# graphcore-research/bess-kge

Measured on AMD Instinct MI355X. Metric: positive+negative triples scored/sec, higher is better.
Workload: dtype f32; 1 GPU; ogbl-biokg-shaped ComplEx d=256 fp32 (W=512), 93,773 entities per shard, n_shard=1, S=4096 positives x 256 per-triple negatives per GPU per step, EmbeddingMoving, mode=score (gather+score+loss); negatives_per_triple=256, mode=score, collectives=none

## Files before the change

bess-kge_amd/csrc/common.h:

```cpp
#pragma once

#include <hip/hip_fp16.h>
#include <hip/hip_runtime.h>
#include <stdint.h>

#include <type_traits>
#include <utility>

#include "../../include/besskge_hip.h"

namespace bess {

int fail(int code, const char* fmt, ...);
int check_launch(const char* what);

#define BESS_REQUIRE(cond, ...)                          \
    do {                                                 \
        if (!(cond)) return ::bess::fail(BESS_EINVAL, __VA_ARGS__); \
    } while (0)

inline hipStream_t as_stream(void* s) { return reinterpret_cast<hipStream_t>(s); }

inline int64_t ceil_div(int64_t a, int64_t b) { return (a + b - 1) / b; }

// ... 75 lines not shown
                   const CountArgs* count = nullptr);

typedef _Float16 half_t;

template <typename T>
__device__ __forceinline__ float to_f32(T v) {
    return static_cast<float>(v);
}

template <typename T, int VEC>
struct VecLoad {
    typedef T vec_t __attribute__((ext_vector_type(VEC)));
    __device__ __forceinline__ static void load(const T* __restrict__ p, float (&out)[VEC]) {
        vec_t v = *reinterpret_cast<const vec_t*>(p);
#pragma unroll
        for (int i = 0; i < VEC; ++i) out[i] = static_cast<float>(v[i]);
    }
};
template <typename T>
struct VecLoad<T, 1> {
    __device__ __forceinline__ static void load(const T* __restrict__ p, float (&out)[1]) {
        out[0] = static_cast<float>(*p);
    }
};

template <typename T, int VEC>
__device__ __forceinline__ void load_chunk(const T* __restrict__ row, int c, int nch, float (&out)[VEC]) {
    VecLoad<T, VEC>::load(row + min(c, nch - 1) * VEC, out);
    const bool live = c < nch;
#pragma unroll
    for (int i = 0; i < VEC; ++i) out[i] = live ? out[i] : 0.f;
}

template <typename T, int VEC>
__device__ __forceinline__ void load_chunk_clamped(const T* __restrict__ row, int c, int nch, float (&out)[VEC]) {
    VecLoad<T, VEC>::load(row + min(c, nch - 1) * VEC, out);
}

__device__ __forceinline__ float row16_allreduce_sum(float v) {
#define BESS_DPP_ROR(x, n)                                                                     \
    __builtin_bit_cast(float, __builtin_amdgcn_update_dpp(0, __builtin_bit_cast(int, (x)),     \
                                                           0x120 | (n), 0xf, 0xf, false))
    v += BESS_DPP_ROR(v, 8);
    v += BESS_DPP_ROR(v, 4);
    v += BESS_DPP_ROR(v, 2);
    v += BESS_DPP_ROR(v, 1);
#undef BESS_DPP_ROR
    return v;
}

__device__ __forceinline__ float wave_allreduce_sum(float v) {
    v = row16_allreduce_sum(v);
    v += __shfl_xor(v, 16, 64);
    v += __shfl_xor(v, 32, 64);
    return v;
}
__device__ __forceinline__ float wave_allreduce_max(float v) {
#pragma unroll
    for (int m = 32; m >= 1; m >>= 1) v = fmaxf(v, __shfl_xor(v, m, 64));
    return v;
}

__device__ __forceinline__ float sgnf(float x) {
    return (x > 0.f) ? 1.f : ((x < 0.f) ? -1.f : 0.f);
}

__device__ __forceinline__ void store_agent(float* p, float v) {
    __hip_atomic_store(p, v, __ATOMIC_RELAXED, __HIP_MEMORY_SCOPE_AGENT);
}
__device__ __forceinline__ float load_agent(const float* p) {
    return __hip_atomic_load(p, __ATOMIC_RELAXED, __HIP_MEMORY_SCOPE_AGENT);
}
__device__ __forceinline__ void release_to_agent() { asm volatile("s_waitcnt vmcnt(0)" ::: "memory"); }
__device__ __forceinline__ bool last_workgroup_ticket(int32_t* counters) {
    const int grid = static_cast<int>(gridDim.x), sub = static_cast<int>(blockIdx.x) & 15;
    const int members = (grid - sub + 15) >> 4;
    int32_t* mine = counters + 32 * (1 + sub);
    if (__hip_atomic_fetch_add(mine, 1, __ATOMIC_RELAXED, __HIP_MEMORY_SCOPE_AGENT) != members - 1) return false;
    __hip_atomic_store(mine, 0, __ATOMIC_RELAXED, __HIP_MEMORY_SCOPE_AGENT);
    if (__hip_atomic_fetch_add(counters, 1, __ATOMIC_RELAXED, __HIP_MEMORY_SCOPE_AGENT) != min(grid, 16) - 1) return false;
    __hip_atomic_store(counters, 0, __ATOMIC_RELAXED, __HIP_MEMORY_SCOPE_AGENT);
    return true;
}


constexpr float SGN_PRESCALE = 1.2676506002282294e30f;
__device__ __forceinline__ float sgn_prescaled(float d_scaled) {
    return __builtin_amdgcn_fmed3f(d_scaled, -1.f, 1.f);
}

struct WordJobs {
    uint32_t* dst[BESS_MAX_WORD_JOBS];
    const uint32_t* src[BESS_MAX_WORD_JOBS];
    uint32_t value[BESS_MAX_WORD_JOBS];
    int64_t first[BESS_MAX_WORD_JOBS + 1];
    int n;
};
__device__ __forceinline__ void run_word_jobs(const WordJobs& J, int block, int n_blocks, int threads) {
    const int64_t total = J.first[J.n];
    const int64_t stride = static_cast<int64_t>(n_blocks) * threads;
    for (int64_t i = static_cast<int64_t>(block) * threads + threadIdx.x; i < total; i += stride) {
        int j = 0;
#pragma unroll
        for (int k = 1; k < BESS_MAX_WORD_JOBS; ++k) j += (k < J.n && i >= J.first[k]) ? 1 : 0;
        const int64_t off = i - J.first[j];
        J.dst[j][off] = J.src[j] ? J.src[j][off] + J.value[j] : J.value[j];
    }
}
int make_word_jobs(int32_t n_jobs, void* const* job_dst, const void* const* job_src, const uint32_t* job_value,
                   const int64_t* job_words, WordJobs* J, int64_t* words, const char* who);

static __global__ __launch_bounds__(256) void k_fill_words(uint32_t* __restrict__ p, uint32_t v, int64_t n) {
    for (int64_t i = blockIdx.x * 256ll + threadIdx.x; i < n; i += 256ll * gridDim.x) p[i] = v;
}
inline hipError_t fill_words_async(void* p, uint32_t v, int64_t n_words, hipStream_t st) {
    if (n_words <= 0) return hipSuccess;
#ifdef BESS_PROBE_MEMSET_NODES
    if (v == 0u || v == 0xffffffffu) return hipMemsetAsync(p, static_cast<int>(v & 0xffu), sizeof(uint32_t) * n_words, st);
#endif
    int64_t blocks = (n_words + 255) / 256;
    blocks = blocks > 2048 ? 2048 : blocks;
    k_fill_words<<<static_cast<unsigned>(blocks), 256, 0, st>>>(static_cast<uint32_t*>(p), v, n_words);
    return hipGetLastError();
}

__device__ __forceinline__ float lp_term(float d, float p) { return p == 2.f ? d * d : powf(fabsf(d), p); }
__device__ __forceinline__ float lp_root(float acc, float p) { return p == 2.f ? sqrtf(acc) : powf(acc, 1.f / p); }
__device__ __forceinline__ float lp_dterm(float d, float p) {
    return p == 2.f ? d : copysignf(powf(fabsf(d), p - 1.f), d);
}
__device__ __forceinline__ float lp_inv(float norm, float p) {
    return norm > 0.f ? (p == 2.f ? 1.f / norm : powf(norm, 1.f - p)) : 0.f;
}

template <typename T>
__device__ __forceinline__ const T* row_ptr(const T* base, const int32_t* idx, int64_t i, int width) {
    const int64_t r = idx ? static_cast<int64_t>(idx[i]) : i;
    return base + r * width;
}

template <typename T_, int VEC_, int IT_>
struct RowClass {
    using T = T_;
    static constexpr int VEC = VEC_, IT = IT_;
};
template <int... V>
using Ints = std::integer_sequence<int, V...>;
struct NativeRows {
    using f32_vecs = Ints<4, 1>;
    using f16_vecs = Ints<8, 2, 1>;
    using its = Ints<1, 2, 4, 8, 16>;
};
struct PartRows {
    using f32_vecs = Ints<4, 1>;
    using f16_vecs = Ints<4, 1>;
    using its = Ints<1, 2, 4, 8>;
};
template <typename T, int VEC, typename F, int... ITS>
bool row_class_by_it(int it, F& f, Ints<ITS...>) {
    return ((it <= ITS ? (f(RowClass<T, VEC, ITS>{}), true) : false) || ...);
}
template <typename T, typename ITS, typename F, int... VECS>
bool row_class_by_vec(int vec, int it, F& f, Ints<VECS...>) {
    return ((vec == VECS && row_class_by_it<T, VECS>(it, f, ITS{})) || ...);
}
template <typename Policy, typename F>
// ... 60 lines not shown
```

bess-kge_amd/csrc/loss.hip:

```cpp
#include "common.h"
#include "loss_rows.h"

namespace bess {

__global__ __launch_bounds__(256) void k_mask_scores(float* __restrict__ neg, int64_t n_triple,
                                                     int64_t n_neg, int64_t ld, int diag_step, int ht,
                                                     int ppp, const uint8_t* __restrict__ mask,
                                                     int64_t mask_rows, int64_t mask_cols) {
    const int64_t total = n_triple * n_neg;
    const int cut = ppp / 2;
    for (int64_t t = blockIdx.x * 256ll + threadIdx.x; t < total; t += 256ll * gridDim.x) {
        const int64_t s = t / n_neg;
        const int64_t j = t - s * n_neg;
        const int64_t blk = ppp > 0 ? s / ppp : 0;
        const int p = ppp > 0 ? static_cast<int>(s - blk * ppp) : 0;
        bool kill = false;
        if (diag_step > 0) {
            const int64_t qpos = ht ? (blk * cut + (p % cut)) : s;
            kill = (j == static_cast<int64_t>(diag_step) * qpos);
        }
        const int64_t mj = j - (n_neg - mask_cols);
        if (mask && mj >= 0) {
            int64_t mrow = s;
            if (mask_rows == 1) mrow = 0;
            else if (mask_rows == 2) mrow = (p >= cut) ? 1 : 0;
            kill = mask[mrow * mask_cols + mj] == 0;
        }
        if (kill) neg[s * ld + j] += BESS_BAD_NEGATIVE_SCORE;
    }
}

template <int KIND, bool ADV, bool GRAD, int CH>
__global__ __launch_bounds__(256) void k_loss_rows(bess_loss_desc l, const float* __restrict__ pos,
                                                   const float* __restrict__ neg, int64_t n_triple,
                                                   int64_t n_neg, int64_t ld_neg,
                                                   const float* __restrict__ weight,
                                                   int64_t weight_len, float* __restrict__ row_loss,
                                                   float* __restrict__ d_pos,
                                                   float* __restrict__ d_neg, int64_t ld_dneg,
                                                   float* __restrict__ row_norm, int32_t* __restrict__ counter,
                                                   float* __restrict__ loss) {
    const int64_t s = blockIdx.x * 4ll + (threadIdx.x >> 6);
    if (s < n_triple)
        loss_row<KIND, ADV, GRAD, CH>(l, pos, neg, s, n_neg, ld_neg, weight, weight_len, row_loss, d_pos, d_neg, ld_dneg,
                                      row_norm);
    if (!counter) return;
    __shared__ float part[256];
    __shared__ int last;
    release_to_agent();
    __syncthreads();
    if (threadIdx.x == 0) last = last_workgroup_ticket(counter);
    __syncthreads();
    if (!last) return;
    float acc = 0.f;
    for (int64_t i = threadIdx.x; i < n_triple; i += 256) acc += load_agent(row_loss + i);
    part[threadIdx.x] = acc;
    __syncthreads();
    for (int h = 128; h > 0; h >>= 1) {
        if (threadIdx.x < h) part[threadIdx.x] += part[threadIdx.x + h];
        __syncthreads();
    }
    if (threadIdx.x == 0) loss[0] = part[0];
}

__global__ __launch_bounds__(256) void k_ranks_from_scores(const float* __restrict__ pos,
                                                           const float* __restrict__ cand, int64_t n_row,
                                                           int64_t n_cand, int64_t ld, int mode, int worst_inf,
                                                           float* __restrict__ rank) {
    const int lane = threadIdx.x & 63;
    const int64_t s = blockIdx.x * 4ll + (threadIdx.x >> 6);
    if (s >= n_row) return;
    float p = pos[s];
    if (p != p) p = -INFINITY;
    const float* row = cand + s * ld;
    float gt = 0.f, ge = 0.f;
    for (int64_t j = lane; j < n_cand; j += 64) {
        const float c = row[j];
        gt += (c > p) ? 1.f : 0.f;
        ge += (c >= p) ? 1.f : 0.f;
    }
    gt = wave_allreduce_sum(gt);
    ge = wave_allreduce_sum(ge);
    if (lane == 0) {
        const float n = static_cast<float>(n_cand);
        float better;
        bool worst;
        if (mode == 0) { better = gt; worst = gt == n; }
        else if (mode == 1) { better = ge; worst = ge == n; }
        else { better = 0.5f * (gt + ge); worst = (gt == n) || (ge == n); }
        rank[s] = (worst_inf && worst) ? INFINITY : 1.f + better;
    }
}

__global__ __launch_bounds__(256) void k_ranks_from_indices(const int64_t* __restrict__ truth,
                                                            const int64_t* __restrict__ cand, int64_t n_row,
                                                            int64_t n_cand, int worst_inf,
                                                            float* __restrict__ rank) {
    const int64_t s = blockIdx.x * 256ll + threadIdx.x;
    if (s >= n_row) return;
    const int64_t t = truth[s];
    float r = worst_inf ? INFINITY : static_cast<float>(n_cand + 1);
    for (int64_t j = n_cand - 1; j >= 0; --j)
        if (cand[s * n_cand + j] == t) r = static_cast<float>(j + 1);
    rank[s] = r;
}

__global__ __launch_bounds__(1024) void k_sum_rows(const float* __restrict__ row_loss, int64_t n,
                                                   float* __restrict__ loss) {
    __shared__ float part[1024];
    float acc = 0.f;
    for (int64_t i = threadIdx.x; i < n; i += 1024) acc += row_loss[i];
    part[threadIdx.x] = acc;
    __syncthreads();
    for (int s = 512; s > 0; s >>= 1) {
        if (threadIdx.x < s) part[threadIdx.x] += part[threadIdx.x + s];
        __syncthreads();
    }
    if (threadIdx.x == 0) loss[0] = part[0];
}

static int loss_chunks(bool grad, const float* neg, int64_t N, int64_t ld, const float* dn, int64_t ldd) {
    const bool vec = N % 4 == 0 && ld % 4 == 0 && reinterpret_cast<uintptr_t>(neg) % 16 == 0 &&
                     (!grad || (ldd % 4 == 0 && reinterpret_cast<uintptr_t>(dn) % 16 == 0));
    if (!vec) return 0;
    if (N > 256 * 24) return -1;
    return N <= 256 * 4 ? 4 : N <= 256 * 12 ? 12 : 24;
}

}

using namespace bess;

extern "C" int bess_mask_scores(float* neg, int64_t n_triple, int64_t n_neg, int64_t ld,
                                int32_t diag_step, int32_t ht, int32_t ppp, const uint8_t* mask,
                                int64_t mask_rows, int64_t mask_cols, void* stream) {
    BESS_REQUIRE(n_triple >= 0 && n_neg >= 0 && ld >= n_neg, "mask_scores: bad sizes");
    if (n_triple == 0 || n_neg == 0) return BESS_OK;
    BESS_REQUIRE(neg, "mask_scores: NULL scores");
    BESS_REQUIRE(diag_step >= 0, "mask_scores: negative diag_step");
// ... 101 lines not shown
```

bess-kge_amd/csrc/prepare.hip:

```cpp
#include "common.h"
#include "loss_rows.h"

namespace bess {

struct TripleArgs {
    const void* head_base;
    const int32_t* head_idx;
    const void* tail_base;
    const int32_t* tail_idx;
    const void* rel_table;
    const int32_t* rel_idx;
    int64_t n;
    int W;
    int Wr;
    int norm_p;
};

template <typename T, int SCORER>
__device__ __forceinline__ void triple_fwd_body(const TripleArgs& a, int64_t s, int lane, float* __restrict__ out) {
    const T* h = row_ptr(static_cast<const T*>(a.head_base), a.head_idx, s, a.W);
    const T* t = row_ptr(static_cast<const T*>(a.tail_base), a.tail_idx, s, a.W);
    const T* r = static_cast<const T*>(a.rel_table) + static_cast<int64_t>(a.rel_idx[s]) * a.Wr;
    float acc = 0.f;
    if (SCORER == BESS_TRANSE) {
        for (int e = lane; e < a.W; e += 64) {
            const float x = to_f32(h[e]) + to_f32(r[e]) - to_f32(t[e]);
            acc += (a.norm_p == 1) ? fabsf(x) : lp_term(x, static_cast<float>(a.norm_p));
        }
    } else if (SCORER == BESS_DISTMULT) {
        for (int e = lane; e < a.W; e += 64) acc += to_f32(h[e]) * to_f32(r[e]) * to_f32(t[e]);
    } else {
        const int d = a.W / 2;
        for (int e = lane; e < d; e += 64) {
            const float hr = to_f32(h[e]), hi = to_f32(h[d + e]);
            const float tr = to_f32(t[e]), ti = to_f32(t[d + e]);
            float rr, ri;
            if (SCORER == BESS_ROTATE) {
                const float ph = to_f32(r[e]);
                rr = cosf(ph);
                ri = sinf(ph);
            } else {
                rr = to_f32(r[e]);
                ri = to_f32(r[d + e]);
            }
            const float qr = hr * rr - hi * ri;
            const float qi = hr * ri + hi * rr;
            if (SCORER == BESS_ROTATE) {
                const float xr = qr - tr, xi = qi - ti;
                acc += (a.norm_p == 1) ? (fabsf(xr) + fabsf(xi))
                                       : (lp_term(xr, static_cast<float>(a.norm_p)) + lp_term(xi, static_cast<float>(a.norm_p)));
            } else {
                acc += qr * tr + qi * ti;
            }
        }
    }
    acc = wave_allreduce_sum(acc);
    if (SCORER == BESS_TRANSE || SCORER == BESS_ROTATE)
        acc = -((a.norm_p == 1) ? acc : lp_root(acc, static_cast<float>(a.norm_p)));
    if (lane == 0) out[s] = acc;
}

template <typename T, int SCORER>
__global__ __launch_bounds__(256) void k_score_triple_fwd(TripleArgs a, float* __restrict__ out) {
    const int lane = threadIdx.x & 63;
    const int64_t s = blockIdx.x * 4ll + (threadIdx.x >> 6);
    if (s >= a.n) return;
    triple_fwd_body<T, SCORER>(a, s, lane, out);
}

struct QueryArgs {
    const void* ent_base;
    const int32_t* ent_idx;
    const void* rel_table;
    const int32_t* rel_idx;
    int64_t n;
    int W;
    int Wr;
    int side;
};

template <typename T, int SCORER>
__device__ __forceinline__ void query_fwd_body(const QueryArgs& a, int64_t q, int lane, float* __restrict__ query) {
    const T* x = row_ptr(static_cast<const T*>(a.ent_base), a.ent_idx, q, a.W);
    const T* r = static_cast<const T*>(a.rel_table) + static_cast<int64_t>(a.rel_idx[q]) * a.Wr;
    float* o = query + q * a.W;
    const bool tail = a.side == BESS_CORRUPT_TAIL;
    if (SCORER == BESS_TRANSE) {
        for (int e = lane; e < a.W; e += 64)
            o[e] = tail ? (to_f32(x[e]) + to_f32(r[e])) : (to_f32(x[e]) - to_f32(r[e]));
    } else if (SCORER == BESS_DISTMULT) {
        for (int e = lane; e < a.W; e += 64) o[e] = to_f32(x[e]) * to_f32(r[e]);
    } else {
        const int d = a.W / 2;
        for (int e = lane; e < d; e += 64) {
            const float xr = to_f32(x[e]), xi = to_f32(x[d + e]);
            float rr, ri;
            if (SCORER == BESS_ROTATE) {
                const float ph = tail ? to_f32(r[e]) : -to_f32(r[e]);
                rr = cosf(ph);
                ri = sinf(ph);
            } else {
                rr = to_f32(r[e]);
                ri = tail ? to_f32(r[d + e]) : -to_f32(r[d + e]);
            }
            o[e] = xr * rr - xi * ri;
            o[d + e] = xr * ri + xi * rr;
        }
    }
}

template <typename T, int SCORER>
__global__ __launch_bounds__(256) void k_query_fwd(QueryArgs a, float* __restrict__ query) {
    const int lane = threadIdx.x & 63;
    const int64_t q = blockIdx.x * 4ll + (threadIdx.x >> 6);
    if (q >= a.n) return;
    query_fwd_body<T, SCORER>(a, q, lane, query);
}

template <typename T, int SCORER>
__global__ __launch_bounds__(256) void k_query_triple_fwd(TripleArgs a, QueryArgs qa, float* __restrict__ query,
                                                          float* __restrict__ out) {
    const int lane = threadIdx.x & 63;
    const int64_t s = blockIdx.x * 4ll + (threadIdx.x >> 6);
    if (s >= a.n) return;
    query_fwd_body<T, SCORER>(qa, s, lane, query);
    triple_fwd_body<T, SCORER>(a, s, lane, out);
}

template <typename T, int SCORER>
__global__ __launch_bounds__(256) void k_query_triple_fwd_jobs(TripleArgs a, QueryArgs qa, float* __restrict__ query,
                                                               float* __restrict__ out, WordJobs J, int triple_blocks) {
    if (static_cast<int>(blockIdx.x) >= triple_blocks) {
        run_word_jobs(J, static_cast<int>(blockIdx.x) - triple_blocks, static_cast<int>(gridDim.x) - triple_blocks, 256);
        return;
    }
    const int lane = threadIdx.x & 63;
    const int64_t s = blockIdx.x * 4ll + (threadIdx.x >> 6);
    if (s >= a.n) return;
    query_fwd_body<T, SCORER>(qa, s, lane, query);
    triple_fwd_body<T, SCORER>(a, s, lane, out);
}

template <bool ACCUM>
__device__ __forceinline__ void put(float* p, float v) {
    if (ACCUM) *p += v;
    else *p = v;
}
template <bool BYROW>
__device__ __forceinline__ void emit(float* p, float v) {
    if (BYROW) {
        if (v != 0.f) unsafeAtomicAdd(p, v);
    } else {
        *p = v;
    }
}
template <bool BYROW, bool ACCUM>
__device__ __forceinline__ void emit2(float* p, float v) {
    if (BYROW) {
        if (v != 0.f) unsafeAtomicAdd(p, v);
    } else {
        put<ACCUM>(p, v);
    }
}

template <typename T, int SCORER, bool BYROW = false>
__device__ __forceinline__ void triple_bwd_body(const TripleArgs& a, int64_t s, int lane,
                                                const float g, float* __restrict__ d_head,
                                                float* __restrict__ d_tail, float* __restrict__ d_rel) {
    const T* h = row_ptr(static_cast<const T*>(a.head_base), a.head_idx, s, a.W);
    const T* t = row_ptr(static_cast<const T*>(a.tail_base), a.tail_idx, s, a.W);
    const int64_t rid = a.rel_idx[s];
    const T* r = static_cast<const T*>(a.rel_table) + rid * a.Wr;
    float* dh = d_head + (BYROW ? (a.head_idx ? static_cast<int64_t>(a.head_idx[s]) : s) : s) * a.W;
    float* dt = d_tail + (BYROW ? (a.tail_idx ? static_cast<int64_t>(a.tail_idx[s]) : s) : s) * a.W;
    float* dr = d_rel + rid * a.Wr;

    if (SCORER == BESS_TRANSE) {
        float inv = 0.f;
        const float pf = static_cast<float>(a.norm_p);
        if (a.norm_p != 1) {
            float ss = 0.f;
            for (int e = lane; e < a.W; e += 64) {
                const float x = to_f32(h[e]) + to_f32(r[e]) - to_f32(t[e]);
                ss += lp_term(x, pf);
            }
            ss = wave_allreduce_sum(ss);
            inv = lp_inv(lp_root(ss, pf), pf);
        }
        for (int e = lane; e < a.W; e += 64) {
            const float x = to_f32(h[e]) + to_f32(r[e]) - to_f32(t[e]);
            const float dx = -g * ((a.norm_p == 1) ? sgnf(x) : lp_dterm(x, pf) * inv);
            emit<BYROW>(dh + e, dx);
            emit<BYROW>(dt + e, -dx);
            if (dx != 0.f) unsafeAtomicAdd(dr + e, dx);
        }
    } else if (SCORER == BESS_DISTMULT) {
        for (int e = lane; e < a.W; e += 64) {
            const float hv = to_f32(h[e]), rv = to_f32(r[e]), tv = to_f32(t[e]);
            emit<BYROW>(dh + e, g * rv * tv);
            emit<BYROW>(dt + e, g * hv * rv);
            unsafeAtomicAdd(dr + e, g * hv * tv);
        }
    } else {
        const int d = a.W / 2;
        float inv = 0.f;
        const float pf = static_cast<float>(a.norm_p);
        if (SCORER == BESS_ROTATE && a.norm_p != 1) {
            float ss = 0.f;
            for (int e = lane; e < d; e += 64) {
                const float hr = to_f32(h[e]), hi = to_f32(h[d + e]);
                const float ph = to_f32(r[e]);
                const float c = cosf(ph), sn = sinf(ph);
                const float xr = hr * c - hi * sn - to_f32(t[e]);
                const float xi = hr * sn + hi * c - to_f32(t[d + e]);
                ss += lp_term(xr, pf) + lp_term(xi, pf);
            }
            ss = wave_allreduce_sum(ss);
            inv = lp_inv(lp_root(ss, pf), pf);
        }
        for (int e = lane; e < d; e += 64) {
            const float hr = to_f32(h[e]), hi = to_f32(h[d + e]);
            const float tr = to_f32(t[e]), ti = to_f32(t[d + e]);
            if (SCORER == BESS_ROTATE) {
// ... 174 lines not shown
                const float riq = sg * ri;
                const float qr = gr * rr + gi * riq, qi = -gr * riq + gi * rr;
                if (tl) vhr += qr, vhi += qi;
                else vtr += qr, vti += qi;
                unsafeAtomicAdd(dr + e, g * (hr * tr + hi * ti) + (gr * xr + gi * xi));
                unsafeAtomicAdd(dr + d + e, g * (-hi * tr + hr * ti) + sg * (-gr * xi + gi * xr));
            }
            emit<BYROW>(dh + e, vhr);
            emit<BYROW>(dh + d + e, vhi);
            emit<BYROW>(dt + e, vtr);
            emit<BYROW>(dt + d + e, vti);
        }
    }
}

template <typename T, int SCORER>
__global__ __launch_bounds__(256) void k_query_bwd(QueryArgs a, const float* __restrict__ d_query,
                                                   float* __restrict__ d_ent,
                                                   float* __restrict__ d_rel) {
    const int lane = threadIdx.x & 63;
    const int64_t q = blockIdx.x * 4ll + (threadIdx.x >> 6);
    if (q >= a.n) return;
    query_bwd_body<T, SCORER, false>(a, q, lane, d_query + q * a.W, d_ent, d_rel);
}

template <typename T, int SCORER>
__global__ __launch_bounds__(256) void k_query_triple_bwd(TripleArgs a, QueryArgs qa, const float* __restrict__ d_out,
                                                          const float* __restrict__ d_query,
                                                          float* __restrict__ d_head, float* __restrict__ d_tail,
                                                          float* __restrict__ d_rel) {
    const int lane = threadIdx.x & 63;
    const int64_t s = blockIdx.x * 4ll + (threadIdx.x >> 6);
    if (s >= a.n) return;
    query_triple_bwd_body<T, SCORER>(a, qa.side, s, lane, d_out[s], d_query + s * qa.W, d_head, d_tail, d_rel);
}

struct TailArgs {
    const float* st_ml;
    const float* st_acc;
    int items;
    bess_loss_desc l;
    const float* pos;
    const float* neg;
    int64_t n_neg, ld_neg;
    const float* weight;
    int64_t weight_len;
    float* row_loss;
    float* loss;
    float* d_pos;
    float* d_neg;
    int64_t ld_dneg;
    float* d_query;
    int32_t* counter;
};

template <typename T, int SCORER, int CH>
__global__ __launch_bounds__(1024) void k_pertriple_tail(TripleArgs a, QueryArgs qa, TailArgs t, float* __restrict__ d_head,
                                                         float* __restrict__ d_tail, float* __restrict__ d_rel) {
    extern __shared__ float tail_lds[];
    __shared__ int last;
    const int lane = threadIdx.x & 63, wv = threadIdx.x >> 6, nw = blockDim.x >> 6;
    const int64_t s = static_cast<int64_t>(blockIdx.x) * nw + wv;
    if (s < a.n) {
        float* row = tail_lds + wv * a.W;
        combine_dq_row(t.st_ml, t.st_acc, s, t.items, a.W, t.l.kind, t.l.loss_scale, t.pos, t.weight, t.weight_len, nullptr,
                       row, t.d_query ? t.d_query + s * a.W : nullptr);
        float g;
#define BESS_TAIL_LOSS(KIND, ADV)                                                                                        \
    g = loss_row_impl<KIND, ADV, true, CH>(t.l, t.pos, t.neg, s, t.n_neg, t.ld_neg, t.weight, t.weight_len, t.row_loss, \
                                           t.d_pos, t.d_neg, t.ld_dneg, nullptr)
        if (t.l.kind == BESS_LOSS_SSCE) BESS_TAIL_LOSS(BESS_LOSS_SSCE, false);
        else if (t.l.kind == BESS_LOSS_LOGSIGMOID && t.l.adversarial) BESS_TAIL_LOSS(BESS_LOSS_LOGSIGMOID, true);
        else if (t.l.kind == BESS_LOSS_LOGSIGMOID) BESS_TAIL_LOSS(BESS_LOSS_LOGSIGMOID, false);
        else if (t.l.adversarial) BESS_TAIL_LOSS(BESS_LOSS_MARGIN, true);
        else BESS_TAIL_LOSS(BESS_LOSS_MARGIN, false);
#undef BESS_TAIL_LOSS
        query_triple_bwd_body<T, SCORER>(a, qa.side, s, lane, g, row, d_head, d_tail, d_rel);
    }
    release_to_agent();
    __syncthreads();
    if (threadIdx.x == 0) last = last_workgroup_ticket(t.counter);
    __syncthreads();
    if (!last) return;
    float acc = 0.f;
    for (int64_t i = threadIdx.x; i < a.n; i += blockDim.x) acc += load_agent(t.row_loss + i);
    tail_lds[threadIdx.x] = acc;
    __syncthreads();
    for (int h = blockDim.x >> 1; h > 0; h >>= 1) {
        if (static_cast<int>(threadIdx.x) < h) tail_lds[threadIdx.x] += tail_lds[threadIdx.x + h];
        __syncthreads();
    }
    if (threadIdx.x == 0) t.loss[0] = tail_lds[0];
}

template <typename T, int SCORER>
__global__ __launch_bounds__(256) void k_query_triple_bwd_parts(TripleArgs a, QueryArgs qa, const float* __restrict__ d_out,
                                                                const float* __restrict__ dq_parts, int n_dq,
                                                                const float* __restrict__ de_parts, int n_de, int64_t n_neg,
                                                                const int32_t* __restrict__ neg_idx,
                                                                float* __restrict__ acc_head, float* __restrict__ acc_tail,
                                                                float* __restrict__ acc_neg, float* __restrict__ d_rel,
                                                                int triple_blocks) {
    extern __shared__ float dq_rows[];
    const int lane = threadIdx.x & 63, wv = threadIdx.x >> 6;
    if (static_cast<int>(blockIdx.x) >= triple_blocks) {
        const int64_t n_wave = (static_cast<int64_t>(gridDim.x) - triple_blocks) * 4;
        for (int64_t j = (static_cast<int64_t>(blockIdx.x) - triple_blocks) * 4 + wv; j < n_neg; j += n_wave) {
            float* dst = acc_neg + static_cast<int64_t>(neg_idx[j]) * a.W;
            if ((a.W & 3) == 0) {
                for (int e = lane * 4; e < a.W; e += 256) {
                    const float* src = de_parts + j * a.W + e;
                    const int64_t slab = n_neg * a.W;
                    float s0 = 0.f, s1 = 0.f, s2 = 0.f, s3 = 0.f;
#pragma unroll 16
                    for (int p = 0; p < n_de; ++p) {
                        const float4 v = *reinterpret_cast<const float4*>(src + p * slab);
                        s0 += v.x, s1 += v.y, s2 += v.z, s3 += v.w;
                    }
                    if (s0 != 0.f) unsafeAtomicAdd(dst + e, s0);
                    if (s1 != 0.f) unsafeAtomicAdd(dst + e + 1, s1);
                    if (s2 != 0.f) unsafeAtomicAdd(dst + e + 2, s2);
                    if (s3 != 0.f) unsafeAtomicAdd(dst + e + 3, s3);
                }
                continue;
            }
            for (int e = lane; e < a.W; e += 64) {
                float sum = 0.f;
                for (int p = 0; p < n_de; ++p) sum += de_parts[(static_cast<int64_t>(p) * n_neg + j) * a.W + e];
                if (sum != 0.f) unsafeAtomicAdd(dst + e, sum);
            }
        }
        return;
    }
    const int64_t s = blockIdx.x * 4ll + wv;
    if (s >= a.n) return;
    float* row = dq_rows + wv * a.W;
    if ((a.W & 3) == 0) {
        const int64_t slab = a.n * a.W;
        for (int e = lane * 4; e < a.W; e += 256) {
            const float* src = dq_parts + s * a.W + e;
            float s0 = 0.f, s1 = 0.f, s2 = 0.f, s3 = 0.f;
#pragma unroll 16
            for (int p = 0; p < n_dq; ++p) {
                const float4 v = *reinterpret_cast<const float4*>(src + p * slab);
                s0 += v.x, s1 += v.y, s2 += v.z, s3 += v.w;
            }
            *reinterpret_cast<float4*>(row + e) = make_float4(s0, s1, s2, s3);
        }
    } else {
        for (int e = lane; e < a.W; e += 64) {
            float sum = 0.f;
            for (int p = 0; p < n_dq; ++p) sum += dq_parts[(static_cast<int64_t>(p) * a.n + s) * a.W + e];
            row[e] = sum;
        }
    }
    query_triple_bwd_body<T, SCORER, true>(a, qa.side, s, lane, d_out[s], row, acc_head, acc_tail, d_rel);
}

static int tail_waves(int64_t n, int W) {
    int nw = n > 1024 ? 16 : 4;
    while (nw > 1 && static_cast<size_t>(nw) * W * sizeof(float) > (32u << 10)) nw >>= 1;
    return nw;
}
static int tail_loss_chunks(int64_t n_neg) { return n_neg <= 1024 ? 4 : 12; }

}

using namespace bess;

// ... 230 lines not shown
```

Before: 5.230 billion triples/s.

## Register-resident forward rows with fused query+triple scoring and unrolled loss tail sum

Restructures the positive-triple and query forward kernels so each wave loads its head, tail and relation row elements into registers with a compile-time trip count, issuing all loads before computing. When both query and triple score are needed, the rows are loaded once and used for both, where previously they were read twice. The last-workgroup loss reduction now issues 16 independent agent-scope loads per iteration to hide latency. Register pressure rises with the unroll depth, and clamped indices read redundant elements.

```diff
diff --git a/bess-kge_amd/csrc/common.h b/bess-kge_amd/csrc/common.h
--- a/bess-kge_amd/csrc/common.h
+++ b/bess-kge_amd/csrc/common.h
@@ -181,6 +181,17 @@
     __hip_atomic_store(counters, 0, __ATOMIC_RELAXED, __HIP_MEMORY_SCOPE_AGENT);
     return true;
 }
+__device__ __forceinline__ float strided_sum_agent(const float* p, int64_t n, int tid, int threads) {
+    float acc = 0.f;
+    for (int64_t i0 = tid; i0 < n; i0 += 16ll * threads) {
+        float v[16];
+#pragma unroll
+        for (int j = 0; j < 16; ++j) v[j] = load_agent(p + min(i0 + static_cast<int64_t>(j) * threads, n - 1));
+#pragma unroll
+        for (int j = 0; j < 16; ++j) acc = (i0 + static_cast<int64_t>(j) * threads < n) ? acc + v[j] : acc;
+    }
+    return acc;
+}
 
 
 constexpr float SGN_PRESCALE = 1.2676506002282294e30f;
diff --git a/bess-kge_amd/csrc/loss.hip b/bess-kge_amd/csrc/loss.hip
--- a/bess-kge_amd/csrc/loss.hip
+++ b/bess-kge_amd/csrc/loss.hip
@@ -52,9 +52,7 @@
     if (threadIdx.x == 0) last = last_workgroup_ticket(counter);
     __syncthreads();
     if (!last) return;
-    float acc = 0.f;
-    for (int64_t i = threadIdx.x; i < n_triple; i += 256) acc += load_agent(row_loss + i);
-    part[threadIdx.x] = acc;
+    part[threadIdx.x] = strided_sum_agent(row_loss, n_triple, threadIdx.x, 256);
     __syncthreads();
     for (int h = 128; h > 0; h >>= 1) {
         if (threadIdx.x < h) part[threadIdx.x] += part[threadIdx.x + h];
diff --git a/bess-kge_amd/csrc/prepare.hip b/bess-kge_amd/csrc/prepare.hip
--- a/bess-kge_amd/csrc/prepare.hip
+++ b/bess-kge_amd/csrc/prepare.hip
@@ -16,48 +16,167 @@
     int norm_p;
 };
 
+constexpr bool is_complex_scorer(int scorer) { return scorer == BESS_ROTATE || scorer == BESS_COMPLEX; }
+
+template <int SCORER>
+__device__ __forceinline__ float triple_term(float hr, float hi, float tr, float ti, float r0, float r1, int norm_p) {
+    if (SCORER == BESS_TRANSE) {
+        const float x = hr + r0 - tr;
+        return (norm_p == 1) ? fabsf(x) : lp_term(x, static_cast<float>(norm_p));
+    } else if (SCORER == BESS_DISTMULT) {
+        return hr * r0 * tr;
+    } else {
+        float rr, ri;
+        if (SCORER == BESS_ROTATE) {
+            rr = cosf(r0);
+            ri = sinf(r0);
+        } else {
+            rr = r0;
+            ri = r1;
+        }
+        const float qr = hr * rr - hi * ri;
+        const float qi = hr * ri + hi * rr;
+        if (SCORER == BESS_ROTATE) {
+            const float xr = qr - tr, xi = qi - ti;
+            return (norm_p == 1) ? (fabsf(xr) + fabsf(xi))
+                                 : (lp_term(xr, static_cast<float>(norm_p)) + lp_term(xi, static_cast<float>(norm_p)));
+        }
+        return qr * tr + qi * ti;
+    }
+}
+
+template <int SCORER>
+__device__ __forceinline__ void query_elem(float xr, float xi, float r0, float r1, bool tail, float& o0, float& o1) {
+    if (SCORER == BESS_TRANSE) {
+        o0 = tail ? (xr + r0) : (xr - r0);
+    } else if (SCORER == BESS_DISTMULT) {
+        o0 = xr * r0;
+    } else {
+        float rr, ri;
+        if (SCORER == BESS_ROTATE) {
+            const float ph = tail ? r0 : -r0;
+            rr = cosf(ph);
+            ri = sinf(ph);
+        } else {
+            rr = r0;
+            ri = tail ? r1 : -r1;
+        }
+        o0 = xr * rr - xi * ri;
+        o1 = xr * ri + xi * rr;
+    }
+}
+
+__device__ __forceinline__ float finish_triple_score(int scorer, float acc, int norm_p) {
+    acc = wave_allreduce_sum(acc);
+    if (scorer == BESS_TRANSE || scorer == BESS_ROTATE)
+        acc = -((norm_p == 1) ? acc : lp_root(acc, static_cast<float>(norm_p)));
+    return acc;
+}
+
+__device__ __forceinline__ int64_t row_id(const int32_t* __restrict__ idx, const int32_t* __restrict__ other, int64_t s) {
+    const int32_t v = (idx ? idx : other)[s];
+    return idx ? static_cast<int64_t>(v) : s;
+}
+
+constexpr int REG_ROW_MAX = 1024;
+template <typename T, int SCORER, int NK, bool QUERY, bool TRIPLE>
+__device__ __forceinline__ void fwd_rows_in_registers(const T* __restrict__ h, const T* __restrict__ t,
+                                                      const T* __restrict__ r, int W, int norm_p, bool tail, int lane,
+                                                      float* __restrict__ o, float* __restrict__ out_s) {
+    constexpr bool CPLX = is_complex_scorer(SCORER);
+    constexpr bool R2 = SCORER == BESS_COMPLEX;
+    const int lim = CPLX ? W / 2 : W;
+    float h0[NK], h1[NK], t0[NK], t1[NK], r0[NK], r1[NK];
+#pragma unroll
+    for (int k = 0; k < NK; ++k) {
+        const int e = min(lane + 64 * k, lim - 1);
+        h0[k] = to_f32(h[e]);
+        h1[k] = CPLX ? to_f32(h[lim + e]) : 0.f;
+        t0[k] = TRIPLE ? to_f32(t[e]) : 0.f;
+        t1[k] = (TRIPLE && CPLX) ? to_f32(t[lim + e]) : 0.f;
+        r0[k] = to_f32(r[e]);
+        r1[k] = R2 ? to_f32(r[lim + e]) : 0.f;
+    }
+    float acc = 0.f;
+#pragma unroll
+    for (int k = 0; k < NK; ++k) {
+        const int e = lane + 64 * k;
+        const bool live = e < lim;
+        if (QUERY) {
+            const bool from_h = !TRIPLE || tail;
+            float q0, q1 = 0.f;
+            query_elem<SCORER>(from_h ? h0[k] : t0[k], from_h ? h1[k] : t1[k], r0[k], r1[k], tail, q0, q1);
+            if (live) {
+                o[e] = q0;
+                if (CPLX) o[lim + e] = q1;
+            }
+        }
+        if (TRIPLE) {
+            const float term = triple_term<SCORER>(h0[k], h1[k], t0[k], t1[k], r0[k], r1[k], norm_p);
+            acc = live ? acc + term : acc;
+        }
+    }
+    if (TRIPLE) {
+        acc = finish_triple_score(SCORER, acc, norm_p);
+        if (lane == 0) *out_s = acc;
+    }
+}
+template <typename T, int SCORER, bool QUERY, bool TRIPLE>
+__device__ __forceinline__ void fwd_rows_by_trips(const T* __restrict__ h, const T* __restrict__ t, const T* __restrict__ r,
+                                                  int W, int norm_p, bool tail, int lane, float* __restrict__ o,
+                                                  float* __restrict__ out_s) {
+    const int lim = is_complex_scorer(SCORER) ? W / 2 : W;
+    if (lim <= 256) {
+        fwd_rows_in_registers<T, SCORER, 4, QUERY, TRIPLE>(h, t, r, W, norm_p, tail, lane, o, out_s);
+    } else if (is_complex_scorer(SCORER) || lim <= 512) {
+        fwd_rows_in_registers<T, SCORER, 8, QUERY, TRIPLE>(h, t, r, W, norm_p, tail, lane, o, out_s);
+    } else {
+        if constexpr (!is_complex_scorer(SCORER))
+            fwd_rows_in_registers<T, SCORER, 16, QUERY, TRIPLE>(h, t, r, W, norm_p, tail, lane, o, out_s);
+    }
+}
+
+template <typename T, int SCORER>
+__device__ __forceinline__ void triple_fwd_loops(const T* __restrict__ h, const T* __restrict__ t, const T* __restrict__ r,
+                                                 int W, int norm_p, int lane, float* __restrict__ out_s) {
+    float acc = 0.f;
+    if (!is_complex_scorer(SCORER)) {
+        for (int e = lane; e < W; e += 64)
+            acc += triple_term<SCORER>(to_f32(h[e]), 0.f, to_f32(t[e]), 0.f, to_f32(r[e]), 0.f, norm_p);
+    } else {
+        const int d = W / 2;
+        for (int e = lane; e < d; e += 64)
+            acc += triple_term<SCORER>(to_f32(h[e]), to_f32(h[d + e]), to_f32(t[e]), to_f32(t[d + e]), to_f32(r[e]),
+                                       SCORER == BESS_COMPLEX ? to_f32(r[d + e]) : 0.f, norm_p);
+    }
+    acc = finish_triple_score(SCORER, acc, norm_p);
+    if (lane == 0) *out_s = acc;
+}
+template <typename T, int SCORER>
+__device__ __forceinline__ void query_fwd_loops(const T* __restrict__ x, const T* __restrict__ r, int W, bool tail, int lane,
+                                                float* __restrict__ o) {
+    if (!is_complex_scorer(SCORER)) {
+        for (int e = lane; e < W; e += 64) {
+            float o1;
+            query_elem<SCORER>(to_f32(x[e]), 0.f, to_f32(r[e]), 0.f, tail, o[e], o1);
+        }
+    } else {
+        const int d = W / 2;
+        for (int e = lane; e < d; e += 64)
+            query_elem<SCORER>(to_f32(x[e]), to_f32(x[d + e]), to_f32(r[e]), SCORER == BESS_COMPLEX ? to_f32(r[d + e]) : 0.f,
+                               tail, o[e], o[d + e]);
+    }
+}
+
 template <typename T, int SCORER>
 __device__ __forceinline__ void triple_fwd_body(const TripleArgs& a, int64_t s, int lane, float* __restrict__ out) {
-    const T* h = row_ptr(static_cast<const T*>(a.head_base), a.head_idx, s, a.W);
-    const T* t = row_ptr(static_cast<const T*>(a.tail_base), a.tail_idx, s, a.W);
-    const T* r = static_cast<const T*>(a.rel_table) + static_cast<int64_t>(a.rel_idx[s]) * a.Wr;
-    float acc = 0.f;
-    if (SCORER == BESS_TRANSE) {
-        for (int e = lane; e < a.W; e += 64) {
-            const float x = to_f32(h[e]) + to_f32(r[e]) - to_f32(t[e]);
-            acc += (a.norm_p == 1) ? fabsf(x) : lp_term(x, static_cast<float>(a.norm_p));
-        }
-    } else if (SCORER == BESS_DISTMULT) {
-        for (int e = lane; e < a.W; e += 64) acc += to_f32(h[e]) * to_f32(r[e]) * to_f32(t[e]);
-    } else {
-        const int d = a.W / 2;
-        for (int e = lane; e < d; e += 64) {
-            const float hr = to_f32(h[e]), hi = to_f32(h[d + e]);
-            const float tr = to_f32(t[e]), ti = to_f32(t[d + e]);
-            float rr, ri;
-            if (SCORER == BESS_ROTATE) {
-                const float ph = to_f32(r[e]);
-                rr = cosf(ph);
-                ri = sinf(ph);
-            } else {
-                rr = to_f32(r[e]);
-                ri = to_f32(r[d + e]);
-            }
-            const float qr = hr * rr - hi * ri;
-            const float qi = hr * ri + hi * rr;
-            if (SCORER == BESS_ROTATE) {
-                const float xr = qr - tr, xi = qi - ti;
-                acc += (a.norm_p == 1) ? (fabsf(xr) + fabsf(xi))
-                                       : (lp_term(xr, static_cast<float>(a.norm_p)) + lp_term(xi, static_cast<float>(a.norm_p)));
-            } else {
-                acc += qr * tr + qi * ti;
-            }
-        }
-    }
-    acc = wave_allreduce_sum(acc);
-    if (SCORER == BESS_TRANSE || SCORER == BESS_ROTATE)
-        acc = -((a.norm_p == 1) ? acc : lp_root(acc, static_cast<float>(a.norm_p)));
-    if (lane == 0) out[s] = acc;
+    const int64_t hid = row_id(a.head_idx, a.rel_idx, s), tid = row_id(a.tail_idx, a.rel_idx, s);
+    const int64_t rid = a.rel_idx[s];
+    const T* h = static_cast<const T*>(a.head_base) + hid * a.W;
+    const T* t = static_cast<const T*>(a.tail_base) + tid * a.W;
+    const T* r = static_cast<const T*>(a.rel_table) + rid * a.Wr;
+    if (a.W <= REG_ROW_MAX) fwd_rows_by_trips<T, SCORER, false, true>(h, t, r, a.W, a.norm_p, false, lane, nullptr, out + s);
+    else triple_fwd_loops<T, SCORER>(h, t, r, a.W, a.norm_p, lane, out + s);
 }
 
 template <typename T, int SCORER>
@@ -81,31 +200,30 @@
 
 template <typename T, int SCORER>
 __device__ __forceinline__ void query_fwd_body(const QueryArgs& a, int64_t q, int lane, float* __restrict__ query) {
-    const T* x = row_ptr(static_cast<const T*>(a.ent_base), a.ent_idx, q, a.W);
-    const T* r = static_cast<const T*>(a.rel_table) + static_cast<int64_t>(a.rel_idx[q]) * a.Wr;
+    const int64_t xid = row_id(a.ent_idx, a.rel_idx, q), rid = a.rel_idx[q];
+    const T* x = static_cast<const T*>(a.ent_base) + xid * a.W;
+    const T* r = static_cast<const T*>(a.rel_table) + rid * a.Wr;
     float* o = query + q * a.W;
     const bool tail = a.side == BESS_CORRUPT_TAIL;
-    if (SCORER == BESS_TRANSE) {
-        for (int e = lane; e < a.W; e += 64)
-            o[e] = tail ? (to_f32(x[e]) + to_f32(r[e])) : (to_f32(x[e]) - to_f32(r[e]));
-    } else if (SCORER == BESS_DISTMULT) {
-        for (int e = lane; e < a.W; e += 64) o[e] = to_f32(x[e]) * to_f32(r[e]);
-    } else {
-        const int d = a.W / 2;
-        for (int e = lane; e < d; e += 64) {
-            const float xr = to_f32(x[e]), xi = to_f32(x[d + e]);
-            float rr, ri;
-            if (SCORER == BESS_ROTATE) {
-                const float ph = tail ? to_f32(r[e]) : -to_f32(r[e]);
-                rr = cosf(ph);
-                ri = sinf(ph);
-            } else {
-                rr = to_f32(r[e]);
-                ri = tail ? to_f32(r[d + e]) : -to_f32(r[d + e]);
-            }
-            o[e] = xr * rr - xi * ri;
-            o[d + e] = xr * ri + xi * rr;
-        }
+    if (a.W <= REG_ROW_MAX) fwd_rows_by_trips<T, SCORER, true, false>(x, x, r, a.W, 0, tail, lane, o, nullptr);
+    else query_fwd_loops<T, SCORER>(x, r, a.W, tail, lane, o);
+}
+
+template <typename T, int SCORER>
+__device__ __forceinline__ void query_triple_fwd_body(const TripleArgs& a, int side, int64_t s, int lane,
+                                                      float* __restrict__ query, float* __restrict__ out) {
+    const int64_t hid = row_id(a.head_idx, a.rel_idx, s), tid = row_id(a.tail_idx, a.rel_idx, s);
+    const int64_t rid = a.rel_idx[s];
+    const T* h = static_cast<const T*>(a.head_base) + hid * a.W;
+    const T* t = static_cast<const T*>(a.tail_base) + tid * a.W;
+    const T* r = static_cast<const T*>(a.rel_table) + rid * a.Wr;
+    const bool tail = side == BESS_CORRUPT_TAIL;
+    float* o = query + s * a.W;
+    if (a.W <= REG_ROW_MAX) {
+        fwd_rows_by_trips<T, SCORER, true, true>(h, t, r, a.W, a.norm_p, tail, lane, o, out + s);
+    } else {
+        query_fwd_loops<T, SCORER>(tail ? h : t, r, a.W, tail, lane, o);
+        triple_fwd_loops<T, SCORER>(h, t, r, a.W, a.norm_p, lane, out + s);
     }
 }
 
@@ -123,8 +241,7 @@
     const int lane = threadIdx.x & 63;
     const int64_t s = blockIdx.x * 4ll + (threadIdx.x >> 6);
     if (s >= a.n) return;
-    query_fwd_body<T, SCORER>(qa, s, lane, query);
-    triple_fwd_body<T, SCORER>(a, s, lane, out);
+    query_triple_fwd_body<T, SCORER>(a, qa.side, s, lane, query, out);
 }
 
 template <typename T, int SCORER>
@@ -137,8 +254,7 @@
     const int lane = threadIdx.x & 63;
     const int64_t s = blockIdx.x * 4ll + (threadIdx.x >> 6);
     if (s >= a.n) return;
-    query_fwd_body<T, SCORER>(qa, s, lane, query);
-    triple_fwd_body<T, SCORER>(a, s, lane, out);
+    query_triple_fwd_body<T, SCORER>(a, qa.side, s, lane, query, out);
 }
 
 template <bool ACCUM>
@@ -479,9 +595,7 @@
     if (threadIdx.x == 0) last = last_workgroup_ticket(t.counter);
     __syncthreads();
     if (!last) return;
-    float acc = 0.f;
-    for (int64_t i = threadIdx.x; i < a.n; i += blockDim.x) acc += load_agent(t.row_loss + i);
-    tail_lds[threadIdx.x] = acc;
+    tail_lds[threadIdx.x] = strided_sum_agent(t.row_loss, a.n, threadIdx.x, blockDim.x);
     __syncthreads();
     for (int h = blockDim.x >> 1; h > 0; h >>= 1) {
         if (static_cast<int>(threadIdx.x) < h) tail_lds[threadIdx.x] += tail_lds[threadIdx.x + h];
```

New measurement: 5.351 billion triples/s, median of 6. +2.3%, better.
